# wzx99/DCFP

Hardware: AMD Instinct MI355X
Metric: training images/sec at 1024x2048 DeepLabv3-R101 (higher is better)
Workload: dtype f32

## Files before the change

dcfp_amd/csrc/conv_igemm.hip:

```cpp
#include "common.h"
#include <string.h>
#include <stdio.h>
#include <stdlib.h>

namespace {

int check_desc(const DcfpConvDesc* d) {
    if (!d) return DCFP_E_BADDESC;
    if (d->N <= 0 || d->Cin <= 0 || d->Cout <= 0 || d->H <= 0 || d->W <= 0 || d->stride <= 0 ||
        d->dil <= 0 || d->pad < 0)
        return DCFP_E_BADDESC;
    if (d->KH != d->KW || (d->KH != 1 && d->KH != 3)) return DCFP_E_UNSUPPORTED;
    const int ho = (d->H + 2 * d->pad - d->dil * (d->KH - 1) - 1) / d->stride + 1;
    const int wo = (d->W + 2 * d->pad - d->dil * (d->KW - 1) - 1) / d->stride + 1;
    if (ho != d->Hout || wo != d->Wout || ho <= 0 || wo <= 0) return DCFP_E_BADDESC;
    if ((d->x_pitch != 0 && (d->x_pitch < d->W || (d->x_pitch & 3))) ||
        (d->dy_pitch != 0 && (d->dy_pitch < d->Wout || (d->dy_pitch & 3))))
        return DCFP_E_BADDESC;
    if ((long long)d->Cin * d->H * (d->x_pitch ? d->x_pitch : d->W) >= (1LL << 29) ||
        (long long)d->Cout * d->Hout * (d->dy_pitch ? d->dy_pitch : d->Wout) >= (1LL << 29) ||
        (long long)d->Cout * d->Cin * d->KH * d->KW >= (1LL << 29))
        return DCFP_E_UNSUPPORTED;
    return DCFP_OK;
}
// ... 13 lines not shown
                    int Hi, int Wi, int Ho, int Wo, int sn, int sd, int off0, int offstep,
                    int accumulate, void* workspace, size_t workspace_bytes, hipStream_t stream,
                    const float* scale = nullptr, const float* shift = nullptr,
                    const float* residual = nullptr, int relu = 0, float* stat_part = nullptr, int wp_valid = 0,
                    int in_pitch = 0, long long wp_nstride = 0, const float* fan_src = nullptr,
                    const unsigned long long* fan_mask = nullptr, const Igemm2Red* red = nullptr);
bool dcfp_wino_ok(int N, int H, int W, int d, int M, int Ck);
size_t dcfp_wino_workspace_bytes(int N, int H, int W, int d, int M, int Ck);
double dcfp_wino_exec_fraction(int N, int H, int W, int d, int M, int Ck);
int dcfp_wino_run(const float* in, long long in_nstride, int in_pitch, const float* w, int sAm, int sAc, int flip,
                  float* out, long long out_nstride, int N, int M, int Ck, int H, int W, int d, int accumulate,
                  void* workspace, size_t workspace_bytes, hipStream_t stream, float* xform_out = nullptr,
                  float* stat_part = nullptr, const float* scale = nullptr, const float* shift = nullptr,
                  const float* residual = nullptr, int relu = 0, int wp_valid = 0);
long long dcfp_wino_stat_slots(int N, int H, int W, int d);
bool dcfp_stem_shape(const DcfpConvDesc* d);
int dcfp_stem_fwd(const DcfpConvDesc* d, const float* x, const float* w, const float* bias, float* y, long long y_nstride,
                  hipStream_t stream, float* stat_part = nullptr);
long long dcfp_stem_stat_slots(const DcfpConvDesc* d, const float* y, long long y_nstride);
bool dcfp_gemv_shape(const DcfpConvDesc* d);
int dcfp_gemv_fwd(const DcfpConvDesc* d, const float* x, const float* w, const float* bias, float* y, long long y_nstride,
                  hipStream_t stream);
int dcfp_gemv_dgrad(const DcfpConvDesc* d, const float* dy, long long dy_nstride, const float* w, float* dx, int accumulate,
                    hipStream_t stream);
bool dcfp_wino_fused_ok(int N, int H, int W, int d, int M, int Ck, long long in_nstride, int pitch);
size_t dcfp_wino_fused_workspace_bytes(int N, int H, int W, int d, int M, int Ck);
void dcfp_wino_fused_pads(int N, int H, int W, int d, int M, int Ck, int* CkP, int* Mpad);
size_t dcfp_wino_xform_bytes(int N, int H, int W, int d, int C);
bool dcfp_wgrad_is_winograd(const DcfpConvDesc* d);
bool dcfp_wgrad_wants_xform(const DcfpConvDesc* d);
long long dcfp_igemm2_stat_slots(int M, int P, int N, long long out_nstride, const float* out);
bool dcfp_igemm2_dma_shape(int T, int M, int Ck, int P, long long px, int sn, int sd, int off0, int HiWi, int Wo);
bool dcfp_igemm2_persist();
void dcfp_igemm2_wp_layout(int T, int M, int Ck, int P, long long px, int sn, int sd, int off0, int offstep, int HiWi,
                           int Wo, bool pitched, int sAm, int sAc, DcfpWpEntry* e);
bool dcfp_igemm2_use_dma8(int T, int M, int P, long long px, int sn, int sd, int off0, int offstep, int HiWi,
                          int Wo, bool pitched);
int dcfp_igemm2_permute_multi(const DcfpWpEntry* table, int n, long long total_blocks, hipStream_t stream);


size_t dcfp_igemm3_workspace_bytes(int T, int M, int Ck);
int dcfp_igemm3_run(const float* in, long long in_nstride, const float* w, int sAm, int sAc,
                    const float* bias, float* out, long long out_nstride, int N, int M, int Ck, int T,
                    int Hi, int Wi, int Ho, int Wo, int off0, int offstep, int accumulate,
                    void* workspace, size_t workspace_bytes, hipStream_t stream,
                    const float* scale = nullptr, const float* shift = nullptr,
                    const float* residual = nullptr, int relu = 0, int wp_valid = 0);
int dcfp_igemm2_cfg_id(int M, long long px, int sd);
static bool math_bf16x3() {
    static const bool v = [] { const char* e = getenv("DCFP_CONV_MATH"); return e && !strcmp(e, "bf16x3"); }();
    return v;
}
static bool igemm3_ok(int M, long long px, int sn, int sd) {
    return math_bf16x3() && sn == 1 && sd == 1 && dcfp_igemm2_cfg_id(M, px, sd) == 4;
}

static int wino_kind(const DcfpConvDesc* d, int pass) {
    static const int mode = [] { const char* e = getenv("DCFP_CONV_WINOGRAD"); return e ? atoi(e) : 1; }();
    if (mode == 0) return 0;
    if (d->KH != 3 || d->KW != 3 || d->stride != 1 || d->pad != d->dil || d->Hout != d->H || d->Wout != d->W)
        return 0;
    if (math_bf16x3()) return 0;
    const bool fwd = pass == DCFP_CONV_FWD;
    const int M = fwd ? d->Cout : d->Cin, Ck = fwd ? d->Cin : d->Cout;
    const int sp = fwd ? d->x_pitch : d->dy_pitch;
    const bool pitched = sp && sp != d->W;
// ... 67 lines not shown
        if (igemm3_ok(d->Cin, px, 1, d->stride)) b3 = dcfp_igemm3_workspace_bytes(T, d->Cin, d->Cout);
    }
    return b2 > b3 ? b2 : b3;
}

extern "C" int dcfp_conv2d_kernel_name(const DcfpConvDesc* d, int pass, char* buf, int buf_len) {
    int rc = check_desc(d);
    if (rc) return rc;
    if (!buf || buf_len <= 0) return DCFP_E_BADDESC;
    if (dcfp_gemv_shape(d)) return snprintf(buf, buf_len, "gemv_1x1_map_kernel");
    if (pass == DCFP_CONV_WGRAD) return dcfp_wgrad_kernel_name(d, buf, buf_len);
    if (pass == DCFP_CONV_FWD && dcfp_stem_shape(d)) return snprintf(buf, buf_len, "stem_fwd_kernel");
    if (const int wk = wino_kind(d, pass))
        return wk == 1 ? snprintf(buf, buf_len, "winograd_f2x2_3x3 (igemm2_dma1p_kernel<false,true>)")
                       : snprintf(buf, buf_len, "winograd_f2x2_3x3 fused (wino_fused_kernel)");
    const int M = pass == DCFP_CONV_FWD ? d->Cout : d->Cin;
    const long long px = pass == DCFP_CONV_FWD ? (long long)d->N * d->Hout * d->Wout : (long long)d->N * d->H * d->W;
    const int sd = pass == DCFP_CONV_FWD ? 1 : d->stride;
    if (igemm3_ok(M, px, pass == DCFP_CONV_FWD ? d->stride : 1, sd))
        return snprintf(buf, buf_len, "igemm3_kernel<%d>", d->KH * d->KW);
    const int P = pass == DCFP_CONV_FWD ? d->Hout * d->Wout : d->H * d->W;
    const int HiWi = pass == DCFP_CONV_FWD ? d->H * d->W : d->Hout * d->Wout;
    const int Ck = pass == DCFP_CONV_FWD ? d->Cin : d->Cout;
    {
        const int sp = pass == DCFP_CONV_FWD ? d->x_pitch : d->dy_pitch;
        const bool pitched = sp && sp != (pass == DCFP_CONV_FWD ? d->W : d->Wout);
        if (dcfp_igemm2_use_dma8(d->KH * d->KW, M, P, px, pass == DCFP_CONV_FWD ? d->stride : 1, sd,
                                 pass == DCFP_CONV_FWD ? -d->pad : d->pad, pass == DCFP_CONV_FWD ? d->dil : -d->dil,
                                 HiWi, pass == DCFP_CONV_FWD ? d->Wout : d->W, pitched))
            return snprintf(buf, buf_len, "igemm2_dma8_kernel<%d>", d->KH * d->KW);
    }
    if (dcfp_igemm2_dma_shape(d->KH * d->KW, M, Ck, P, px, pass == DCFP_CONV_FWD ? d->stride : 1, sd, d->pad, HiWi,
                              pass == DCFP_CONV_FWD ? d->Wout : d->W)) {
        if (d->KH == 1 && dcfp_igemm2_persist()) return snprintf(buf, buf_len, "igemm2_dma1p_kernel");
        const int src_pitch = pass == DCFP_CONV_FWD ? d->x_pitch : d->dy_pitch;
        const bool pitched = src_pitch && src_pitch != (pass == DCFP_CONV_FWD ? d->W : d->Wout);
        return snprintf(buf, buf_len, "igemm2_dma_kernel<%d,%s>", d->KH * d->KW,
                        (d->KH == 3 && ((d->pad | d->dil) & 3) != 0 && !pitched) ? "true" : "false");
    }
    return snprintf(buf, buf_len, "igemm2_kernel<%d,%s>", d->KH * d->KW, dcfp_igemm2_cfg_args(M, px, sd));
}

extern "C" double dcfp_conv2d_executed_fraction(const DcfpConvDesc* d, int pass) {
    if (check_desc(d) != DCFP_OK) return 1.0;
    if (pass == DCFP_CONV_WGRAD) return dcfp_wgrad_exec_fraction(d);
    const bool fwd = pass == DCFP_CONV_FWD;
    if (wino_pass(d, pass))
        return fwd ? dcfp_wino_exec_fraction(d->N, d->H, d->W, d->dil, d->Cout, d->Cin)
                   : dcfp_wino_exec_fraction(d->N, d->H, d->W, d->dil, d->Cin, d->Cout);
    const int M = fwd ? d->Cout : d->Cin;
    const long long px = fwd ? (long long)d->N * d->Hout * d->Wout : (long long)d->N * d->H * d->W;
    if (igemm3_ok(M, px, fwd ? d->stride : 1, fwd ? 1 : d->stride)) return 1.0;
    const int sp = fwd ? d->x_pitch : d->dy_pitch;
    const bool pitched = sp && sp != (fwd ? d->W : d->Wout);
    return fwd ? dcfp_igemm2_exec_fraction(d->KH * d->KW, d->Cout, d->Cin, d->N, d->H, d->W, d->Hout, d->Wout, d->stride, 1,
                                           -d->pad, d->dil, pitched)
               : dcfp_igemm2_exec_fraction(d->KH * d->KW, d->Cin, d->Cout, d->N, d->Hout, d->Wout, d->H, d->W, 1, d->stride,
                                           d->pad, -d->dil, pitched);
}

extern "C" int64_t dcfp_conv2d_fwd_stat_slots(const DcfpConvDesc* d, const float* y, int64_t y_nstride);

extern "C" size_t dcfp_conv2d_xform_bytes(const DcfpConvDesc* d) {
    if (check_desc(d) != DCFP_OK) return 0;
    if (!wino_pass(d, DCFP_CONV_FWD) || !dcfp_wgrad_wants_xform(d)) return 0;
    return dcfp_wino_xform_bytes(d->N, d->H, d->W, d->dil, d->Cin);
// ... 238 lines not shown
```

dcfp_amd/csrc/conv_igemm2.hip:

```cpp
#include "igemm2_common.h"
#include <queue>
#include <vector>
#include <stdio.h>
#include <stdlib.h>

namespace {

__device__ __forceinline__ int wp_row(int m, int perm8) {
    if (!perm8) return m;
    const int j = m & 255;
    return (m & ~255) + 32 * (j & 7) + (j >> 3);
}

__global__ void __launch_bounds__(256)
permute_weights_kernel(const float* __restrict__ w, float* __restrict__ wp, int T, int Ck, int CkP,
                       int M, int Mpad, int sAm, int sAc, int perm8) {
    const long long total = (long long)T * CkP * Mpad;
    for (long long i = (long long)blockIdx.x * 256 + threadIdx.x; i < total;
         i += (long long)gridDim.x * 256) {
        const int m = wp_row((int)(i % Mpad), perm8);
        const long long r = i / Mpad;
        const int c = (int)(r % CkP);
        const int t = (int)(r / CkP);
        float v = 0.f;
// ... 5 lines not shown
constexpr int kWpBlockElems = DCFP_WP_BLOCK_ELEMS;
__global__ void __launch_bounds__(256)
permute_weights_multi_kernel(const DcfpWpEntry* __restrict__ table, int n) {
    const long long blk = blockIdx.x;
    int lo = 0, hi = n - 1;
    while (lo < hi) {
        const int mid = (lo + hi + 1) >> 1;
        if (table[mid].first_block <= blk) lo = mid; else hi = mid - 1;
    }
    const DcfpWpEntry e = table[lo];
    const long long base = (blk - e.first_block) * kWpBlockElems;
    if (e.perm8 >= 2) {
        const long long pairs = (long long)e.CkP * e.Mpad;
#pragma unroll 1
        for (int u = 0; u < kWpBlockElems / 256; ++u) {
            const long long i = base + u * 256 + threadIdx.x;
            if (i >= pairs) return;
            wino_filter2_pair(e.w, e.sAm, e.sAc, e.perm8 == 3, e.M, e.Ck, e.Mpad, i, e.wp);
        }
        return;
    }
    const long long total = (long long)e.T * e.CkP * e.Mpad;
#pragma unroll
    for (int u = 0; u < kWpBlockElems / 256; ++u) {
        const long long i = base + u * 256 + threadIdx.x;
        if (i >= total) return;
        const int m = wp_row((int)(i % e.Mpad), e.perm8);
        const long long r = i / e.Mpad;
        const int c = (int)(r % e.CkP);
        const int t = (int)(r / e.CkP);
        float v = 0.f;
        if (m < e.M && c < e.Ck) v = e.w[(long long)m * e.sAm + (long long)c * e.sAc + t];
        e.wp[i] = v;
    }
}

__device__ __forceinline__ float half_xor(float v, int mask) {
    switch (mask) {
        case 1: return __builtin_bit_cast(float, __builtin_amdgcn_ds_swizzle(__builtin_bit_cast(int, v), (1 << 10) | 0x1f));
        case 2: return __builtin_bit_cast(float, __builtin_amdgcn_ds_swizzle(__builtin_bit_cast(int, v), (2 << 10) | 0x1f));
        case 4: return __builtin_bit_cast(float, __builtin_amdgcn_ds_swizzle(__builtin_bit_cast(int, v), (4 << 10) | 0x1f));
        case 8: return __builtin_bit_cast(float, __builtin_amdgcn_ds_swizzle(__builtin_bit_cast(int, v), (8 << 10) | 0x1f));
        default: return __builtin_bit_cast(float, __builtin_amdgcn_ds_swizzle(__builtin_bit_cast(int, v), (16 << 10) | 0x1f));
    }
}

template <int TAPS, int TM, int TN, int WM, int WN, bool SD, bool ACC, int KB = 16>
__global__ void __launch_bounds__(64 * WM * WN, (TM * TN <= 8 && WM * WN == 4 && !ACC) ? 2 : 1)
igemm2_kernel(const Igemm2Params p) {
    constexpr int BK = KB;
    constexpr int NPART = BK / 4;
    constexpr int BM = WM * TM * 32, BN = WN * TN * 32, NT = 64 * WM * WN;
    constexpr int AX = BM / 4;
    constexpr int AROWS = (NT / AX) < BK ? (NT / AX) : BK;
    constexpr int APASS = BK / AROWS;
    constexpr int TX = BN / 4, TY = NT / TX, RPT = BK / TY;
    static_assert(APASS >= 1 && APASS * AROWS == BK, "A loader shape");
    static_assert(TY >= 1 && RPT >= 1 && TY * RPT == BK, "B loader shape");

    extern __shared__ __attribute__((aligned(16))) float smem[];
    float* As = smem;
    float* Bs = smem + 2 * BK * BM;

    const int group = 8 * p.tiles_m;
    const int g = blockIdx.x / group, local = blockIdx.x - g * group;
    const int nt = g * 8 + (local & 7);
    const int mt = local >> 3;
    if (nt >= p.tiles_n_total) return;
    const int img = nt / p.tiles_per_img;
    const int ti_img = nt - img * p.tiles_per_img;
    const int phase = SD ? (p.zfold ? p.zfold - 1 : ti_img / p.tiles_per_phase) : 0;
    const int ph_h = SD ? phase / p.sd : 0, ph_w = SD ? phase - ph_h * p.sd : 0;
    const int p0 = (SD && !p.zfold ? ti_img - phase * p.tiles_per_phase : ti_img) * BN;
    const int m0 = mt * BM;

    const int tid = threadIdx.x;
// ... 171 lines not shown
                if constexpr (kk == BK / 2 - 1) store_b(cur ^ 1);
            }
            static_for<0, TM>([&](auto i_) {
                constexpr int i = decltype(i_)::value;
                static_for<0, TN>([&](auto j_) {
                    constexpr int j = decltype(j_)::value;
                    acc[i][j] = __builtin_amdgcn_mfma_f32_32x32x2f32(af[fc][i], bf[fc][j], acc[i][j], 0, 0, 0);
                });
            });
#ifdef DCFP_SGB
            static_for<0, TM * TN>([&](auto) {
                __builtin_amdgcn_sched_group_barrier(0x008, 1, 0);
                __builtin_amdgcn_sched_group_barrier(0x096, DCFP_SGB, 0);
            });
#endif
            __builtin_amdgcn_sched_barrier(0);
        });
        __syncthreads();
    }

    float* o_img = p.out + (long long)img * p.out_nstride;
    if constexpr (TN == 4) {
        if (!SD && m0 + BM <= p.M && p0 + BN <= p.P && p.vec_store && !p.bias && !p.scale && !p.relu) {
            constexpr unsigned kMaxRec = 0x7ffffffcu;
            const __amdgpu_buffer_rsrc_t o_rsrc = __builtin_amdgcn_make_buffer_rsrc(
                o_img + (long long)m0 * p.P + p0, 0, kMaxRec, 0x00020000);
            unsigned voff = (unsigned)((wm * (TM * 32) + TM * 4 * lhi) * p.P + wn * (TN * 32) + TN * l31) * 4u;
            asm volatile("" : "+v"(voff));
            const unsigned P4 = (unsigned)p.P * 4u;
            if constexpr (!ACC) {
                if (p.stat_part) {
                    float* sp = p.stat_part +
                                ((long long)(nt * WN + wn) * p.M + m0 + wm * (TM * 32) + TM * 4 * lhi) * 2;
                    static_for<0, TM>([&](auto i_) {
                        constexpr int i = decltype(i_)::value;
                        float sm[16], q[16];
                        static_for<0, 16>([&](auto r_) {
                            constexpr int r = decltype(r_)::value;
                            sm[r] = (acc[i][0][r] + acc[i][1][r]) + (acc[i][2][r] + acc[i][3][r]);
                        });
                        static_for<0, 5>([&](auto st_) {
                            constexpr int mask = 1 << decltype(st_)::value;
                            static_for<0, 16>([&](auto r_) { constexpr int r = decltype(r_)::value; sm[r] += half_xor(sm[r], mask); });
                        });
                        static_for<0, 16>([&](auto r_) {
                            constexpr int r = decltype(r_)::value;
                            sm[r] *= (1.0f / 128.0f);
                            const float d0 = acc[i][0][r] - sm[r], d1 = acc[i][1][r] - sm[r];
                            const float d2 = acc[i][2][r] - sm[r], d3 = acc[i][3][r] - sm[r];
                            q[r] = (d0 * d0 + d1 * d1) + (d2 * d2 + d3 * d3);
                        });
                        static_for<0, 5>([&](auto st_) {
                            constexpr int mask = 1 << decltype(st_)::value;
                            static_for<0, 16>([&](auto r_) { constexpr int r = decltype(r_)::value; q[r] += half_xor(q[r], mask); });
                        });
                        if (l31 == 0) {
                            static_for<0, 16>([&](auto r_) {
                                constexpr int r = decltype(r_)::value;
                                constexpr int row = TM * ((r & 3) + 8 * (r >> 2)) + i;
                                sp[row * 2] = sm[r]; sp[row * 2 + 1] = q[r];
                            });
                        }
                    });
                }
            }
            static_for<0, TM>([&](auto i_) {
                constexpr int i = decltype(i_)::value;
                f32x4 old[16];
                if constexpr (ACC) {
                    static_for<0, 16>([&](auto r_) {
                        constexpr int r = decltype(r_)::value;
                        constexpr int row = TM * ((r & 3) + 8 * (r >> 2)) + i;
                        old[r] = __builtin_bit_cast(f32x4, __builtin_amdgcn_raw_buffer_load_b128(
                            o_rsrc, voff, (unsigned)row * P4, 0));
                    });
                    __builtin_amdgcn_sched_barrier(0);
                }
                static_for<0, 16>([&](auto r_) {
                    constexpr int r = decltype(r_)::value;
                    constexpr int row = TM * ((r & 3) + 8 * (r >> 2)) + i;
                    f32x4 v = {acc[i][0][r], acc[i][1][r], acc[i][2][r], acc[i][3][r]};
                    if constexpr (ACC) v += old[r];
                    __builtin_amdgcn_raw_buffer_store_b128(__builtin_bit_cast(
                        __attribute__((__vector_size__(4 * sizeof(unsigned)))) unsigned, v),
                        o_rsrc, voff + (unsigned)row * P4, 0, 0);
                });
                if constexpr (ACC) __builtin_amdgcn_sched_barrier(0);
            });
            return;
        }
    }
    int pix = p0 + wn * (TN * 32) + TN * l31;
    asm volatile("" : "+v"(pix));
    if constexpr (SD) {
        int foff[TN];
#pragma unroll
// ... 612 lines not shown
    if (!d8 && !dcfp_igemm2_dma_shape(T, M, Ck, Ho * Wo, px, sn, sd, off0, Hi * Wi, Wo)) return 1.0;
    Igemm2Params p = {};
    p.N = N; p.Hi = Hi; p.Wi = Wi; p.Ho = Ho; p.Wo = Wo; p.P = Ho * Wo; p.off0 = off0; p.offstep = offstep;
    p.tiles_per_img = (p.P + 255) / 256; p.tiles_n_total = p.tiles_per_img * N; p.tiles_m = (M + 255) / 256;
    {
        static const int t2d = [] { const char* e = getenv("DCFP_IGEMM_2D"); return e ? atoi(e) : 5; }();
        const bool fits = (t2d == 4 || t2d == 5) && Hi % (256 >> t2d) == 0 && Wi % (1 << t2d) == 0;
        p.tile2d = (!d8 && fits && !pitched && ((off0 | offstep) & 3) != 0 && Ho == Hi && Wo == Wi) ? t2d : 0;
    }
    if (pick_tapskip(p, 256) == 0) return 1.0;
    long long live = 0;
    for (int ti = 0; ti < p.tiles_per_img; ++ti) live += tile_live_rows(p, ti);
    return (double)live / (3.0 * p.tiles_per_img);
}

void dcfp_igemm2_wp_layout(int T, int M, int Ck, int P, long long px, int sn, int sd, int off0, int offstep, int HiWi,
                           int Wo, bool pitched, int sAm, int sAc, DcfpWpEntry* e) {
    const TileCfg c = pick_cfg(M, px, sd);
    const bool d8 = dcfp_igemm2_use_dma8(T, M, P, px, sn, sd, off0, offstep, HiWi, Wo, pitched);
    e->T = T; e->Ck = Ck; e->CkP = round_up(Ck, ck_pad()); e->M = M; e->Mpad = round_up(M, d8 ? 256 : c.bm);
    e->sAm = sAm; e->sAc = sAc; e->perm8 = d8 ? 1 : 0;
}

int dcfp_igemm2_permute_multi(const DcfpWpEntry* table, int n, long long total_blocks, hipStream_t stream) {
    hipLaunchKernelGGL(permute_weights_multi_kernel, dim3((unsigned)total_blocks), dim3(256), 0, stream, table, n);
    DCFP_RETURN_LAUNCH();
}

bool dcfp_igemm2_persist() {
    static const bool persist = [] { const char* e = getenv("DCFP_IGEMM_PERSIST"); return !e || atoi(e) != 0; }();
    return persist;
}

bool dcfp_igemm2_dma_shape(int T, int M, int Ck, int P, long long px, int sn, int sd, int off0, int HiWi, int Wo) {
    static const bool dma = [] { const char* e = getenv("DCFP_IGEMM_DMA"); return !e || atoi(e) != 0; }();
    static const bool dma9 = [] { const char* e = getenv("DCFP_IGEMM_DMA9"); return !e || atoi(e) != 0; }();
    if (!dma || pick_cfg(M, px, sd).id != 4 || sn != 1 || sd != 1 || HiWi != P || Wo % 4 != 0) return false;
    return T == 1 ? off0 == 0 : dma9;
}

int dcfp_igemm2_run(const float* in, long long in_nstride, const float* w, int sAm, int sAc,
                    const float* bias, float* out, long long out_nstride, int N, int M, int Ck, int T,
                    int Hi, int Wi, int Ho, int Wo, int sn, int sd, int off0, int offstep,
                    int accumulate, void* workspace, size_t workspace_bytes, hipStream_t stream,
                    const float* scale, const float* shift, const float* residual, int relu,
                    float* stat_part, int wp_valid, int in_pitch, long long wp_nstride, const float* fan_src,
                    const unsigned long long* fan_mask, const Igemm2Red* red) {
    const long long px = (long long)N * Ho * Wo;
    const TileCfg c = pick_cfg(M, px, sd);
    Igemm2Params p;
    p.stat_part = stat_part;
    p.wp_nstride = wp_nstride;
    p.fan_src = fan_src; p.fan_mask = fan_mask;
    p.red_x = red ? red->x : nullptr; p.red_mask = red ? red->mask : nullptr;
    p.red_mean = red ? red->mean : nullptr; p.red_part = red ? red->part : nullptr;
    if (red && !fan_src) return DCFP_E_BADDESC;
    p.in = in; p.bias = bias; p.out = out;
    p.scale = scale; p.shift = shift; p.residual = residual; p.relu = relu;
    p.in_nstride = in_nstride; p.out_nstride = out_nstride;
    p.N = N; p.M = M; p.Ck = Ck; p.CkP = round_up(Ck, ck_pad()); p.Mpad = round_up(M, c.bm);
    const bool plain = !scale && !relu && !stat_part;
    const bool d8 = plain && !wp_nstride && !fan_src && dcfp_igemm2_use_dma8(T, M, Ho * Wo, px, sn, sd, off0, offstep, Hi * Wi, Wo,
                                                                 in_pitch > 0 && in_pitch != Wi);
    if (d8) p.Mpad = round_up(M, 256);
    p.Hi = Hi; p.Wi = Wi; p.Ho = Ho; p.Wo = Wo; p.P = Ho * Wo;
    p.in_pitch = in_pitch > 0 ? in_pitch : Wi;
    const bool pitched = p.in_pitch != Wi;
    if (pitched) {
        const int reach = off0 < 0 ? -off0 : off0;
        if (T != 9 || p.in_pitch < Wi + reach || off0 + 2 * offstep != -off0 || (p.in_pitch & 3) ||
// ... 76 lines not shown
```

dcfp_amd/csrc/conv_igemm2p.hip:

```cpp
#include "igemm2_common.h"
#include <stdlib.h>

namespace {

typedef unsigned u32x4 __attribute__((vector_size(16)));
typedef __attribute__((address_space(3))) void* lds_ptr;

__device__ __forceinline__ u32x4 make_desc(const void* base, unsigned bytes) {
    const unsigned long long a = (unsigned long long)base;
    u32x4 d = {(unsigned)a, (unsigned)(a >> 32) & 0xffffu, bytes, 0x00020000u};
    return d;
}

constexpr int kStatFloats = 4 * 64 * 33 * 2;
constexpr int kStatFloats2 = 4 * 32 * 32 * 2;

template <bool ACC, bool WPI = false, int TM_ = 4, bool FAN = false, bool RED = false>
__global__ void __launch_bounds__(256, TM_ == 2 ? 2 : 1) igemm2_dma1p_kernel(const Igemm2Params p, int total_tiles, int dbg) {
    constexpr int TM = TM_, TN = 4, WN = 2, BM = 64 * TM_, BN = 256;
    extern __shared__ __attribute__((aligned(16))) float smem[];
    float* As = smem;
    float* Bs = smem + 2 * BK * BM;
    float* Ss = smem + 2 * BK * (BM + BN);
    const int tid = threadIdx.x;
    const int lane = tid & 63, wid = tid >> 6;
    const int wm = wid / WN, wn = wid - wm * WN;
    const int l31 = lane & 31, lhi = lane >> 5;
    const int HiWi = p.Hi * p.Wi;
    const int group = 8 * p.tiles_m;
    const int nk = p.CkP / BK;

    const int wid_s = __builtin_amdgcn_readfirstlane(wid);
    const unsigned lane16 = lane * 16u;
    const unsigned a2_voff = (unsigned)((lane >> 5) * p.Mpad) * 4u + (unsigned)(lane & 31) * 16u;
    const u32x4 a_desc = make_desc(p.wp, 0x7ffffffcu);
    const unsigned lds_a0 = (unsigned)(size_t)(lds_ptr)As, lds_b0 = (unsigned)(size_t)(lds_ptr)Bs;

    auto decode = [&](int t, int& nt, int& mt) {
        const int g = t / group, local = t - g * group;
        nt = g * 8 + (local & 7);
        mt = local >> 3;
    };
    auto next_valid = [&](int t) {
        while (t < total_tiles) {
            int nt, mt;
            decode(t, nt, mt);
            if (nt < p.tiles_n_total) break;
            t += gridDim.x;
        }
        return t;
    };

    int ld_tile = next_valid(blockIdx.x), ld_cb = 0;
    unsigned ld_boff4 = 0;
    unsigned a_run = 0, b_run = 0;
    u32x4 ld_bdesc = a_desc;
    const unsigned a_row = (unsigned)p.Mpad * 4u, b_row = (unsigned)HiWi * 4u;
    const unsigned a_kstep = (unsigned)(BK * p.Mpad) * 4u, b_kstep = (unsigned)(BK * HiWi) * 4u;
    const unsigned lds_a_w = __builtin_amdgcn_readfirstlane(lds_a0 + (unsigned)(4 * wid_s * BM) * 4u);
    const unsigned lds_b_w = __builtin_amdgcn_readfirstlane(lds_b0 + (unsigned)(4 * wid_s * BN) * 4u);
    auto ld_set_tile = [&]() {
        int nt, mt;
        decode(ld_tile, nt, mt);
        const int img = nt / p.tiles_per_img;
        const int p0 = (nt - img * p.tiles_per_img) * BN;
        a_run = __builtin_amdgcn_readfirstlane((unsigned)(mt * BM + (WPI ? img * (int)p.wp_nstride : 0)) * 4u +
                                               (unsigned)(4 * wid_s) * a_row);
        b_run = __builtin_amdgcn_readfirstlane((unsigned)(4 * wid_s) * b_row);
        ld_bdesc = make_desc(p.in + (long long)img * p.in_nstride, (unsigned)(p.Ck * HiWi) * 4u);
        const int pp = p0 + 4 * lane;
        ld_boff4 = pp < p.P ? (unsigned)pp * 4u : kOob;
    };
    auto issue_piece = [&](unsigned abuf, unsigned bbuf, auto piece_) {
        constexpr int piece = decltype(piece_)::value;
        constexpr int q = piece >> 1;
        if constexpr ((piece & 1) == 0) {
            if constexpr (TM == 4) {
                const unsigned a_s = a_run + (unsigned)q * a_row;
                const unsigned av = lane16;
                const u32x4 ad = a_desc;
                asm volatile("s_add_i32 m0, %0, %4\n\ts_nop 0\n\tbuffer_load_dwordx4 %1, %2, %3 offen lds"
                             :: "s"(abuf), "v"(av), "s"(ad), "s"(a_s), "i"(q * BM * 4) : "memory", "m0", "scc");
            } else if constexpr (q < 2) {
                const unsigned a_s = a_run + (unsigned)(2 * q) * a_row;
                const unsigned av = a2_voff;
                const u32x4 ad = a_desc;
                asm volatile("s_add_i32 m0, %0, %4\n\ts_nop 0\n\tbuffer_load_dwordx4 %1, %2, %3 offen lds"
                             :: "s"(abuf), "v"(av), "s"(ad), "s"(a_s), "i"(2 * q * BM * 4) : "memory", "m0", "scc");
            }
        } else {
            const unsigned b_cb = b_run + (unsigned)q * b_row;
            const unsigned b_s = 0;
            const unsigned bv = ld_boff4 + b_cb;
            const u32x4 bd = ld_bdesc;
            asm volatile("s_add_i32 m0, %0, %4\n\ts_nop 0\n\tbuffer_load_dwordx4 %1, %2, %3 offen lds"
                         :: "s"(bbuf), "v"(bv), "s"(bd), "s"(b_s), "i"(q * BN * 4) : "memory", "m0", "scc");
        }
    };
    auto ld_advance = [&]() {
        a_run += a_kstep;
        b_run += b_kstep;
        if (++ld_cb == nk) {
            ld_cb = 0;
            ld_tile = next_valid(ld_tile + gridDim.x);
            if (ld_tile < total_tiles) ld_set_tile();
        }
    };
    auto issue = [&](int buf) {
        const unsigned abuf = lds_a_w + (buf ? (unsigned)(BK * BM) * 4u : 0u), bbuf = lds_b_w + (buf ? (unsigned)(BK * BN) * 4u : 0u);
        static_for<0, 8>([&](auto piece_) { issue_piece(abuf, bbuf, piece_); });
        ld_advance();
    };
    auto retire = [&]() {
        asm volatile("s_waitcnt vmcnt(0) lgkmcnt(0)" ::: "memory");
        __builtin_amdgcn_s_barrier();
    };

    int tile = ld_tile;
    if (tile >= total_tiles) return;
#ifdef DCFP_P_DEBUG
    if (dbg & 0xff00) {
// ... 47 lines not shown
                    });
                });
                __builtin_amdgcn_sched_barrier(0);
            });
            retire();
            cur ^= 1;
        }

        float* o_img = p.out + (long long)img * p.out_nstride;
#ifdef DCFP_P_DEBUG
        if (dbg & 1) {
            if (acc[0][0][0] == 123.456f) o_img[0] = 1.f;
            tile = next_tile;
            continue;
        }
#endif
        if (m0 + BM > p.M || p0 + BN > p.P) {
            int pix = p0 + wn * (TN * 32) + TN * l31;
            asm volatile("" : "+v"(pix));
#pragma unroll
            for (int i = 0; i < TM; ++i) {
#pragma unroll
                for (int r = 0; r < 16; ++r) {
                    const int row = (r & 3) + 8 * (r >> 2) + 4 * lhi;
                    const int m = m0 + wm * (TM * 32) + TM * row + i;
                    if (m >= p.M || pix >= p.P) continue;
                    float* dst = o_img + (long long)m * p.P + pix;
                    f32x4 v = {acc[i][0][r], acc[i][1][r], acc[i][2][r], acc[i][3][r]};
                    if constexpr (ACC) v += *reinterpret_cast<const f32x4*>(dst);
                    *reinterpret_cast<f32x4*>(dst) = v;
                }
            }
        } else {
            if constexpr (!ACC && TM == 4) {
                if (p.stat_part) {
                    typedef float f32x2 __attribute__((ext_vector_type(2)));
                    f32x2* st = reinterpret_cast<f32x2*>(Ss) + wid * (64 * 33);
                    float* sp = p.stat_part + ((long long)(nt * WN + wn) * p.M + m0 + wm * (TM * 32)) * 2;
                    static_for<0, 2>([&](auto h_) {
                        constexpr int half = decltype(h_)::value;
                        static_for<0, 2>([&](auto ii_) {
                            constexpr int ii = decltype(ii_)::value;
                            constexpr int i = 2 * half + ii;
                            static_for<0, 16>([&](auto r_) {
                                constexpr int r = decltype(r_)::value;
                                const float a0 = acc[i][0][r], a1 = acc[i][1][r], a2 = acc[i][2][r], a3 = acc[i][3][r];
                                const float s4 = (a0 + a1) + (a2 + a3);
                                const float mu = 0.25f * s4;
                                const float d0 = a0 - mu, d1 = a1 - mu, d2 = a2 - mu, d3 = a3 - mu;
                                f32x2 v = {s4, (d0 * d0 + d1 * d1) + (d2 * d2 + d3 * d3)};
                                st[(lhi * 32 + ii * 16 + r) * 33 + l31] = v;
                            });
                        });
                        float S = 0.f, M2 = 0.f;
#pragma unroll
                        for (int k = 0; k < 32; ++k) {
                            const f32x2 v = st[lane * 33 + k];
                            S += v.x; M2 += v.y;
                        }
                        const float mean = S * (1.0f / 128.0f);
                        __builtin_amdgcn_sched_barrier(0);
#pragma unroll
                        for (int k = 0; k < 32; ++k) {
                            const float d = 0.25f * st[lane * 33 + k].x - mean;
                            M2 += 4.0f * d * d;
                        }
                        const int rr = lane & 15;
                        const int row = 16 * (lane >> 5) + 4 * (rr & 3) + 32 * (rr >> 2) + 2 * half + ((lane >> 4) & 1);
                        sp[row * 2] = mean;
                        sp[row * 2 + 1] = M2;
                    });
                }
            }
            if constexpr (!ACC && TM == 2 && !FAN) {
                if (p.stat_part) {
                    typedef float f32x2 __attribute__((ext_vector_type(2)));
                    f32x2* st = reinterpret_cast<f32x2*>(Ss) + wid * (32 * 32);
                    float* sp = p.stat_part + ((long long)(nt * WN + wn) * p.M + m0 + wm * (TM * 32)) * 2;
                    static_for<0, 2>([&](auto i_) {
                        constexpr int i = decltype(i_)::value;
                        static_for<0, 16>([&](auto r_) {
                            constexpr int r = decltype(r_)::value;
                            const float a0 = acc[i][0][r], a1 = acc[i][1][r], a2 = acc[i][2][r], a3 = acc[i][3][r];
                            const float s4 = (a0 + a1) + (a2 + a3);
                            const float mu = 0.25f * s4;
                            const float d0 = a0 - mu, d1 = a1 - mu, d2 = a2 - mu, d3 = a3 - mu;
                            f32x2 v = {s4, (d0 * d0 + d1 * d1) + (d2 * d2 + d3 * d3)};
                            const int row = lhi * 16 + r;
                            st[row * 32 + ((l31 + row) & 31)] = v;
                        });
                        const int rw = lane & 31;
                        float S = 0.f, M2 = 0.f;
#pragma unroll
                        for (int k = 0; k < 32; ++k) {
                            const f32x2 v = st[rw * 32 + ((k + rw) & 31)];
                            S += v.x; M2 += v.y;
                        }
                        const float mean = S * (1.0f / 128.0f);
                        __builtin_amdgcn_sched_barrier(0);
#pragma unroll
                        for (int k = 0; k < 32; ++k) {
                            const float d = 0.25f * st[rw * 32 + ((k + rw) & 31)].x - mean;
                            M2 += 4.0f * d * d;
                        }
                        if (lane < 32) {
                            const int rr = lane & 15;
                            const int row = 2 * ((rr & 3) + 8 * (rr >> 2) + 4 * (lane >> 4)) + i;
// ... 125 lines not shown
                            o_rsrc, voff + (unsigned)row * P4, 0, 0);
                    else if (p.nt_store == 1)
                        __builtin_amdgcn_raw_buffer_store_b128(__builtin_bit_cast(u4, v), o_rsrc, voff + (unsigned)row * P4, 0, 2);
                    else
                        __builtin_amdgcn_raw_buffer_store_b128(__builtin_bit_cast(u4, v), o_rsrc, voff + (unsigned)row * P4, 0, 18);
                });
                if constexpr (ACC) __builtin_amdgcn_sched_barrier(0);
            });
        }
        tile = next_tile;
    }
}

}

static int p128_mode() {
    static const int p128 = [] { const char* e = getenv("DCFP_IGEMM_P128"); return e ? atoi(e) : 2; }();
    return p128;
}
bool dcfp_igemm2p_fan_red_ok(int Mpad, int CkP) {
    return Mpad % 256 == 0 && (p128_mode() == 2 || (p128_mode() == 1 && CkP <= 256));
}

int dcfp_igemm2p_launch(const Igemm2Params& p, hipStream_t stream) {
    static int cus = 0;
    if (cus == 0) {
        int dev = 0, v = 0;
        if (hipGetDevice(&dev) == hipSuccess &&
            hipDeviceGetAttribute(&v, hipDeviceAttributeMultiprocessorCount, dev) == hipSuccess && v > 0)
            cus = v;
        else
            cus = 256;
    }
    const int p128 = p128_mode();
    static const int half_stats = [] { const char* e = getenv("DCFP_IGEMM_P128_STATS"); return e ? atoi(e) : 2; }();
    const bool k_ok = p128 == 2 || (p128 == 1 && p.CkP <= 256);
    const bool half = p.Mpad % 256 == 0 &&
                      (p.stat_part ? (!p.accumulate && !p.fan_src && !p.wp_nstride && (half_stats == 2 || (half_stats == 1 && k_ok)))
                                   : k_ok);
    Igemm2Params q = p;
    if (half) q.tiles_m = p.tiles_m * 2;
    const long long groups = ((long long)p.tiles_n_total + 7) / 8;
    const long long total = groups * 8 * q.tiles_m;
    if (total > 0x7fffffffLL) return DCFP_E_UNSUPPORTED;
    const long long slots = half ? 2LL * cus : cus;
    long long blocks = total < slots ? total : slots;
    int dbg = 0;
#ifdef DCFP_P_DEBUG
    if (const char* e = getenv("DCFP_DBG_P_BLOCKS")) blocks = atoll(e) < blocks ? atoll(e) : blocks;
    if (const char* e = getenv("DCFP_DBG_P")) dbg = atoi(e);
#endif
    blocks = blocks / 8 * 8;
    if (blocks < 8) blocks = total < 8 ? total : 8;
    const size_t lds = (size_t)(2 * BK * (half ? 384 : 512) + (p.stat_part ? (half ? kStatFloats2 : kStatFloats) : 0)) * sizeof(float);
    auto launch = [&](auto kern) -> int {
        hipError_t e = hipFuncSetAttribute(reinterpret_cast<const void*>(kern),
                                           hipFuncAttributeMaxDynamicSharedMemorySize, (int)lds);
        if (e != hipSuccess) return (int)e;
        hipLaunchKernelGGL(kern, dim3((unsigned)blocks), dim3(256), lds, stream, q, (int)total, dbg);
        DCFP_RETURN_LAUNCH();
    };
    if (p.wp_nstride) {
        if (p.accumulate) return DCFP_E_UNSUPPORTED;
        return half ? launch(igemm2_dma1p_kernel<false, true, 2>) : launch(igemm2_dma1p_kernel<false, true>);
    }
    if (p.fan_src) {
// ... 12 lines not shown
```

dcfp_amd/csrc/igemm2_common.h:

```cpp
#pragma once
#include "common.h"
#include <type_traits>

struct Igemm2Params {
    const float* in;
    const float* wp;
    const float* bias;
    const float* scale;
    const float* shift;
    const float* residual;
    int relu;
    float* out;
    long long in_nstride, out_nstride;
    int N, M, Mpad, Ck, CkP;
    int Hi, Wi, Ho, Wo, P, tiles_per_img, tiles_n_total, tiles_m;
    int sn, sd, off0, offstep;
    int accumulate, vec_store;
    int tile2d;
    int Hc, Wc, tiles_per_phase;
    int in_pitch;
    int zfold;
    const float* fan_src;
    const unsigned long long* fan_mask;
    long long wp_nstride;
// ... 26 lines not shown
                                                  int Mpad, long long idx, float* __restrict__ Ug) {
    const int mblocks = Mpad / 64;
    const int c = (int)(idx / Mpad), m = (int)(idx - (long long)c * Mpad);
    float g[9];
    if (m < M && c < Ck) {
        const float* src = w + (long long)m * sAm + (long long)c * sAc;
#pragma unroll
        for (int t = 0; t < 9; ++t) g[t] = src[flip ? 8 - t : t];
    } else {
#pragma unroll
        for (int t = 0; t < 9; ++t) g[t] = 0.f;
    }
    float r[4][3];
#pragma unroll
    for (int k = 0; k < 3; ++k) {
        const float g0 = g[k], g1 = g[3 + k], g2 = g[6 + k];
        r[0][k] = g0;
        r[1][k] = 0.5f * ((g0 + g2) + g1);
        r[2][k] = 0.5f * ((g0 + g2) - g1);
        r[3][k] = g2;
    }
    const int cb = c >> 3, cl = c & 7, mb = m >> 6, ml = m & 63;
    float* dst = Ug + ((((long long)(cb * mblocks + mb) * 16) * 2 + (ml >> 5)) * 64 + (cl & 1) * 32 + (ml & 31)) * 4 + (cl >> 1);
#pragma unroll
    for (int i = 0; i < 4; ++i) {
        const float a = r[i][0], b = r[i][1], cc = r[i][2];
        dst[(4 * i + 0) * 512] = a;
        dst[(4 * i + 1) * 512] = 0.5f * ((a + cc) + b);
        dst[(4 * i + 2) * 512] = 0.5f * ((a + cc) - b);
        dst[(4 * i + 3) * 512] = cc;
    }
}

template <int T>
struct Frag;
template <>
struct Frag<4> {
    static __device__ __forceinline__ void ld(const float* p, float (&f)[4]) {
        const float4 v = *reinterpret_cast<const float4*>(p);
        f[0] = v.x; f[1] = v.y; f[2] = v.z; f[3] = v.w;
    }
};
template <>
struct Frag<2> {
    static __device__ __forceinline__ void ld(const float* p, float (&f)[2]) {
        const float2 v = *reinterpret_cast<const float2*>(p);
        f[0] = v.x; f[1] = v.y;
    }
};
template <>
struct Frag<1> {
    static __device__ __forceinline__ void ld(const float* p, float (&f)[1]) { f[0] = p[0]; }
};

}
```

Baseline: 12.24.

## Route narrow 1x1 convs (M=64/128) to persistent DMA kernel with narrow tiles

Adds a narrow variant of the persistent DMA 1x1 conv kernel with 64- or 128-row M tiles for layers with 64 or 128 output channels. Previously these shapes went to the generic igemm2 path. It also moves the butterfly stats reduction into a shared helper so the narrow kernel can fuse BN statistics, and it raises occupancy hints (3 workgroups per CU for TM=1). The risks are poorer MFMA reuse with small M tiles and extra template instances.

```diff
diff --git a/dcfp_amd/csrc/conv_igemm.hip b/dcfp_amd/csrc/conv_igemm.hip
--- a/dcfp_amd/csrc/conv_igemm.hip
+++ b/dcfp_amd/csrc/conv_igemm.hip
@@ -69,6 +69,7 @@
 long long dcfp_igemm2_stat_slots(int M, int P, int N, long long out_nstride, const float* out);
 bool dcfp_igemm2_dma_shape(int T, int M, int Ck, int P, long long px, int sn, int sd, int off0, int HiWi, int Wo);
 bool dcfp_igemm2_persist();
+bool dcfp_igemm2_narrow(int T, int M, long long px, int sd);
 void dcfp_igemm2_wp_layout(int T, int M, int Ck, int P, long long px, int sn, int sd, int off0, int offstep, int HiWi,
                            int Wo, bool pitched, int sAm, int sAc, DcfpWpEntry* e);
 bool dcfp_igemm2_use_dma8(int T, int M, int P, long long px, int sn, int sd, int off0, int offstep, int HiWi,
@@ -202,6 +203,8 @@
     }
     if (dcfp_igemm2_dma_shape(d->KH * d->KW, M, Ck, P, px, pass == DCFP_CONV_FWD ? d->stride : 1, sd, d->pad, HiWi,
                               pass == DCFP_CONV_FWD ? d->Wout : d->W)) {
+        if (dcfp_igemm2_narrow(d->KH * d->KW, M, px, sd))
+            return snprintf(buf, buf_len, "igemm2_dma1p_kernel<narrow,%d>", M);
         if (d->KH == 1 && dcfp_igemm2_persist()) return snprintf(buf, buf_len, "igemm2_dma1p_kernel");
         const int src_pitch = pass == DCFP_CONV_FWD ? d->x_pitch : d->dy_pitch;
         const bool pitched = src_pitch && src_pitch != (pass == DCFP_CONV_FWD ? d->W : d->Wout);
diff --git a/dcfp_amd/csrc/conv_igemm2.hip b/dcfp_amd/csrc/conv_igemm2.hip
--- a/dcfp_amd/csrc/conv_igemm2.hip
+++ b/dcfp_amd/csrc/conv_igemm2.hip
@@ -61,16 +61,6 @@
         float v = 0.f;
         if (m < e.M && c < e.Ck) v = e.w[(long long)m * e.sAm + (long long)c * e.sAc + t];
         e.wp[i] = v;
-    }
-}
-
-__device__ __forceinline__ float half_xor(float v, int mask) {
-    switch (mask) {
-        case 1: return __builtin_bit_cast(float, __builtin_amdgcn_ds_swizzle(__builtin_bit_cast(int, v), (1 << 10) | 0x1f));
-        case 2: return __builtin_bit_cast(float, __builtin_amdgcn_ds_swizzle(__builtin_bit_cast(int, v), (2 << 10) | 0x1f));
-        case 4: return __builtin_bit_cast(float, __builtin_amdgcn_ds_swizzle(__builtin_bit_cast(int, v), (4 << 10) | 0x1f));
-        case 8: return __builtin_bit_cast(float, __builtin_amdgcn_ds_swizzle(__builtin_bit_cast(int, v), (8 << 10) | 0x1f));
-        default: return __builtin_bit_cast(float, __builtin_amdgcn_ds_swizzle(__builtin_bit_cast(int, v), (16 << 10) | 0x1f));
     }
 }
 
@@ -308,36 +298,7 @@
                 if (p.stat_part) {
                     float* sp = p.stat_part +
                                 ((long long)(nt * WN + wn) * p.M + m0 + wm * (TM * 32) + TM * 4 * lhi) * 2;
-                    static_for<0, TM>([&](auto i_) {
-                        constexpr int i = decltype(i_)::value;
-                        float sm[16], q[16];
-                        static_for<0, 16>([&](auto r_) {
-                            constexpr int r = decltype(r_)::value;
-                            sm[r] = (acc[i][0][r] + acc[i][1][r]) + (acc[i][2][r] + acc[i][3][r]);
-                        });
-                        static_for<0, 5>([&](auto st_) {
-                            constexpr int mask = 1 << decltype(st_)::value;
-                            static_for<0, 16>([&](auto r_) { constexpr int r = decltype(r_)::value; sm[r] += half_xor(sm[r], mask); });
-                        });
-                        static_for<0, 16>([&](auto r_) {
-                            constexpr int r = decltype(r_)::value;
-                            sm[r] *= (1.0f / 128.0f);
-                            const float d0 = acc[i][0][r] - sm[r], d1 = acc[i][1][r] - sm[r];
-                            const float d2 = acc[i][2][r] - sm[r], d3 = acc[i][3][r] - sm[r];
-                            q[r] = (d0 * d0 + d1 * d1) + (d2 * d2 + d3 * d3);
-                        });
-                        static_for<0, 5>([&](auto st_) {
-                            constexpr int mask = 1 << decltype(st_)::value;
-                            static_for<0, 16>([&](auto r_) { constexpr int r = decltype(r_)::value; q[r] += half_xor(q[r], mask); });
-                        });
-                        if (l31 == 0) {
-                            static_for<0, 16>([&](auto r_) {
-                                constexpr int r = decltype(r_)::value;
-                                constexpr int row = TM * ((r & 3) + 8 * (r >> 2)) + i;
-                                sp[row * 2] = sm[r]; sp[row * 2 + 1] = q[r];
-                            });
-                        }
-                    });
+                    stats_bfly<TM>(acc, sp, l31);
                 }
             }
             static_for<0, TM>([&](auto i_) {
@@ -1016,10 +977,18 @@
     return persist;
 }
 
+bool dcfp_igemm2_narrow(int T, int M, long long px, int sd) {
+    static const bool on = [] { const char* e = getenv("DCFP_IGEMM_NARROW"); return !e || atoi(e) != 0; }();
+    if (!on || T != 1 || sd != 1 || deep_k() || !dcfp_igemm2_persist()) return false;
+    const int id = pick_cfg(M, px, sd).id;
+    return (id == 1 && M == 64) || (id == 2 && M == 128);
+}
+
 bool dcfp_igemm2_dma_shape(int T, int M, int Ck, int P, long long px, int sn, int sd, int off0, int HiWi, int Wo) {
     static const bool dma = [] { const char* e = getenv("DCFP_IGEMM_DMA"); return !e || atoi(e) != 0; }();
     static const bool dma9 = [] { const char* e = getenv("DCFP_IGEMM_DMA9"); return !e || atoi(e) != 0; }();
-    if (!dma || pick_cfg(M, px, sd).id != 4 || sn != 1 || sd != 1 || HiWi != P || Wo % 4 != 0) return false;
+    if (!dma || sn != 1 || sd != 1 || HiWi != P || Wo % 4 != 0) return false;
+    if (pick_cfg(M, px, sd).id != 4) return dcfp_igemm2_narrow(T, M, px, sd) && off0 == 0;
     return T == 1 ? off0 == 0 : dma9;
 }
 
diff --git a/dcfp_amd/csrc/conv_igemm2p.hip b/dcfp_amd/csrc/conv_igemm2p.hip
--- a/dcfp_amd/csrc/conv_igemm2p.hip
+++ b/dcfp_amd/csrc/conv_igemm2p.hip
@@ -15,8 +15,10 @@
 constexpr int kStatFloats = 4 * 64 * 33 * 2;
 constexpr int kStatFloats2 = 4 * 32 * 32 * 2;
 
-template <bool ACC, bool WPI = false, int TM_ = 4, bool FAN = false, bool RED = false>
-__global__ void __launch_bounds__(256, TM_ == 2 ? 2 : 1) igemm2_dma1p_kernel(const Igemm2Params p, int total_tiles, int dbg) {
+template <bool ACC, bool WPI = false, int TM_ = 4, bool FAN = false, bool RED = false, bool NARROW = false>
+__global__ void __launch_bounds__(256, TM_ == 1 ? 3 : TM_ == 2 ? 2 : 1)
+igemm2_dma1p_kernel(const Igemm2Params p, int total_tiles, int dbg) {
+    static_assert(TM_ != 1 || NARROW, "64-row tiles: narrow instances only");
     constexpr int TM = TM_, TN = 4, WN = 2, BM = 64 * TM_, BN = 256;
     extern __shared__ __attribute__((aligned(16))) float smem[];
     float* As = smem;
@@ -32,7 +34,8 @@
 
     const int wid_s = __builtin_amdgcn_readfirstlane(wid);
     const unsigned lane16 = lane * 16u;
-    const unsigned a2_voff = (unsigned)((lane >> 5) * p.Mpad) * 4u + (unsigned)(lane & 31) * 16u;
+    const unsigned a2_voff = TM == 1 ? (unsigned)((lane >> 4) * p.Mpad) * 4u + (unsigned)(lane & 15) * 16u
+                                     : (unsigned)((lane >> 5) * p.Mpad) * 4u + (unsigned)(lane & 31) * 16u;
     const u32x4 a_desc = make_desc(p.wp, 0x7ffffffcu);
     const unsigned lds_a0 = (unsigned)(size_t)(lds_ptr)As, lds_b0 = (unsigned)(size_t)(lds_ptr)Bs;
 
@@ -81,12 +84,18 @@
                 const u32x4 ad = a_desc;
                 asm volatile("s_add_i32 m0, %0, %4\n\ts_nop 0\n\tbuffer_load_dwordx4 %1, %2, %3 offen lds"
                              :: "s"(abuf), "v"(av), "s"(ad), "s"(a_s), "i"(q * BM * 4) : "memory", "m0", "scc");
-            } else if constexpr (q < 2) {
+            } else if constexpr (TM == 2 && q < 2) {
                 const unsigned a_s = a_run + (unsigned)(2 * q) * a_row;
                 const unsigned av = a2_voff;
                 const u32x4 ad = a_desc;
                 asm volatile("s_add_i32 m0, %0, %4\n\ts_nop 0\n\tbuffer_load_dwordx4 %1, %2, %3 offen lds"
                              :: "s"(abuf), "v"(av), "s"(ad), "s"(a_s), "i"(2 * q * BM * 4) : "memory", "m0", "scc");
+            } else if constexpr (TM == 1 && q == 0) {
+                const unsigned a_s = a_run;
+                const unsigned av = a2_voff;
+                const u32x4 ad = a_desc;
+                asm volatile("s_add_i32 m0, %0, %4\n\ts_nop 0\n\tbuffer_load_dwordx4 %1, %2, %3 offen lds"
+                             :: "s"(abuf), "v"(av), "s"(ad), "s"(a_s), "i"(0) : "memory", "m0", "scc");
             }
         } else {
             const unsigned b_cb = b_run + (unsigned)q * b_row;
@@ -200,6 +209,12 @@
                 }
             }
         } else {
+            if constexpr (!ACC && NARROW) {
+                if (p.stat_part) {
+                    float* sp = p.stat_part + ((long long)(nt * WN + wn) * p.M + m0 + wm * (TM * 32) + TM * 4 * lhi) * 2;
+                    stats_bfly<TM>(acc, sp, l31);
+                }
+            }
             if constexpr (!ACC && TM == 4) {
                 if (p.stat_part) {
                     typedef float f32x2 __attribute__((ext_vector_type(2)));
@@ -240,7 +255,7 @@
                     });
                 }
             }
-            if constexpr (!ACC && TM == 2 && !FAN) {
+            if constexpr (!ACC && TM == 2 && !FAN && !NARROW) {
                 if (p.stat_part) {
                     typedef float f32x2 __attribute__((ext_vector_type(2)));
                     f32x2* st = reinterpret_cast<f32x2*>(Ss) + wid * (32 * 32);
@@ -432,6 +447,31 @@
         else
             cus = 256;
     }
+    if (p.Mpad < 256) {
+        if (p.wp_nstride || p.fan_src || (p.Mpad != 64 && p.Mpad != 128) || p.tiles_m != 1) return DCFP_E_UNSUPPORTED;
+        const int wg_per_cu = p.Mpad == 64 ? 3 : 2;
+        Igemm2Params q = p;
+        q.tiles_per_img = (p.P + 255) / 256;
+        q.tiles_n_total = q.tiles_per_img * p.N;
+        const long long total = ((long long)q.tiles_n_total + 7) / 8 * 8;
+        if (total > 0x7fffffffLL) return DCFP_E_UNSUPPORTED;
+        long long blocks = total < (long long)wg_per_cu * cus ? total : (long long)wg_per_cu * cus;
+        blocks = blocks / 8 * 8;
+        if (blocks < 8) blocks = total < 8 ? total : 8;
+        const size_t lds = (size_t)2 * BK * (p.Mpad + 256) * sizeof(float);
+        auto launch = [&](auto kern) -> int {
+            hipError_t e = hipFuncSetAttribute(reinterpret_cast<const void*>(kern),
+                                               hipFuncAttributeMaxDynamicSharedMemorySize, (int)lds);
+            if (e != hipSuccess) return (int)e;
+            hipLaunchKernelGGL(kern, dim3((unsigned)blocks), dim3(256), lds, stream, q, (int)total, 0);
+            DCFP_RETURN_LAUNCH();
+        };
+        if (p.Mpad == 64)
+            return p.accumulate ? launch(igemm2_dma1p_kernel<true, false, 1, false, false, true>)
+                                : launch(igemm2_dma1p_kernel<false, false, 1, false, false, true>);
+        return p.accumulate ? launch(igemm2_dma1p_kernel<true, false, 2, false, false, true>)
+                            : launch(igemm2_dma1p_kernel<false, false, 2, false, false, true>);
+    }
     const int p128 = p128_mode();
     static const int half_stats = [] { const char* e = getenv("DCFP_IGEMM_P128_STATS"); return e ? atoi(e) : 2; }();
     const bool k_ok = p128 == 2 || (p128 == 1 && p.CkP <= 256);
diff --git a/dcfp_amd/csrc/igemm2_common.h b/dcfp_amd/csrc/igemm2_common.h
--- a/dcfp_amd/csrc/igemm2_common.h
+++ b/dcfp_amd/csrc/igemm2_common.h
@@ -82,6 +82,50 @@
     }
 }
 
+__device__ __forceinline__ float half_xor(float v, int mask) {
+    switch (mask) {
+        case 1: return __builtin_bit_cast(float, __builtin_amdgcn_ds_swizzle(__builtin_bit_cast(int, v), (1 << 10) | 0x1f));
+        case 2: return __builtin_bit_cast(float, __builtin_amdgcn_ds_swizzle(__builtin_bit_cast(int, v), (2 << 10) | 0x1f));
+        case 4: return __builtin_bit_cast(float, __builtin_amdgcn_ds_swizzle(__builtin_bit_cast(int, v), (4 << 10) | 0x1f));
+        case 8: return __builtin_bit_cast(float, __builtin_amdgcn_ds_swizzle(__builtin_bit_cast(int, v), (8 << 10) | 0x1f));
+        default: return __builtin_bit_cast(float, __builtin_amdgcn_ds_swizzle(__builtin_bit_cast(int, v), (16 << 10) | 0x1f));
+    }
+}
+
+template <int TM>
+__device__ __forceinline__ void stats_bfly(const f32x16 (&acc)[TM][4], float* sp, int l31) {
+    static_for<0, TM>([&](auto i_) {
+        constexpr int i = decltype(i_)::value;
+        float sm[16], q[16];
+        static_for<0, 16>([&](auto r_) {
+            constexpr int r = decltype(r_)::value;
+            sm[r] = (acc[i][0][r] + acc[i][1][r]) + (acc[i][2][r] + acc[i][3][r]);
+        });
+        static_for<0, 5>([&](auto st_) {
+            constexpr int mask = 1 << decltype(st_)::value;
+            static_for<0, 16>([&](auto r_) { constexpr int r = decltype(r_)::value; sm[r] += half_xor(sm[r], mask); });
+        });
+        static_for<0, 16>([&](auto r_) {
+            constexpr int r = decltype(r_)::value;
+            sm[r] *= (1.0f / 128.0f);
+            const float d0 = acc[i][0][r] - sm[r], d1 = acc[i][1][r] - sm[r];
+            const float d2 = acc[i][2][r] - sm[r], d3 = acc[i][3][r] - sm[r];
+            q[r] = (d0 * d0 + d1 * d1) + (d2 * d2 + d3 * d3);
+        });
+        static_for<0, 5>([&](auto st_) {
+            constexpr int mask = 1 << decltype(st_)::value;
+            static_for<0, 16>([&](auto r_) { constexpr int r = decltype(r_)::value; q[r] += half_xor(q[r], mask); });
+        });
+        if (l31 == 0) {
+            static_for<0, 16>([&](auto r_) {
+                constexpr int r = decltype(r_)::value;
+                constexpr int row = TM * ((r & 3) + 8 * (r >> 2)) + i;
+                sp[row * 2] = sm[r]; sp[row * 2 + 1] = q[r];
+            });
+        }
+    });
+}
+
 template <int T>
 struct Frag;
 template <>
```

After: 12.26, median of 6. Within noise of the previous version (+0.2%).
